# arkworks-rs/groth16

Measured on AMD Instinct MI355X. Metric: R1CS constraints/sec (create_proof, BLS12-381), higher is better.
Workload: dtype u32-limb Montgomery integers (Fr 255-bit, Fq 381-bit); 1 GPU; SYN(k=22) synthetic R1CS, 4194302 constraints, FFT domain 2^22, bls12_381, full create_proof (7 NTTs + 4 G1 MSMs + 1 G2 MSM), valid proving key generated on the GPU from seeded toxic waste; curve=bls12_381, log2_domain=22, constraints=4194302, key=valid, witness=resident in HBM at entry (--full: value_incl_h2d holds the PCIe-inclusive rates), parallelism=single-gpu

## Files before the change

### groth16_amd/csrc/internal.hpp

```cpp
#pragma once
#include <hip/hip_runtime.h>
#include <atomic>
#include <cstdint>
#include <cstdio>
#include <cstring>
#include <string>
#include <vector>
#include "../../include/g16_mi355x.h"
#include "curve.hpp"

namespace g16 {

void set_last_error(const char* what, hipError_t e, const char* file, int line);

#define G16_HIP_TRY(expr)                                                     \
    do {                                                                      \
        hipError_t e__ = (expr);                                              \
        if (e__ != hipSuccess) {                                              \
            ::g16::set_last_error(#expr, e__, __FILE__, __LINE__);            \
            return e__ == hipErrorOutOfMemory ? G16_ERR_OOM : G16_ERR_HIP;    \
        }                                                                     \
    } while (0)

#define G16_TRY(expr)                  \
    do {                               \
        int rc__ = (expr);             \
        if (rc__ != G16_OK) return rc__; \
    } while (0)

#define G16_LAUNCH_CHECK() G16_HIP_TRY(hipGetLastError())

struct PerDeviceOnce {
    std::atomic<bool> done[64] = {};
    std::atomic<bool>& flag() {
        int dev = 0;
        (void)hipGetDevice(&dev);
        return done[dev & 63];
    }
};

struct Arena {
    struct Chunk { char* p; size_t cap; size_t used; };
    std::vector<Chunk> chunks;
    size_t min_chunk = (size_t)256 << 20;
    void reset() { for (auto& c : chunks) c.used = 0; }
    int alloc(size_t bytes, void** out);
    template <class T> int alloc_n(size_t n, T** out) { return alloc(n * sizeof(T), (void**)out); }
    void release();
    size_t total() const { size_t t = 0; for (auto& c : chunks) t += c.cap; return t; }
};

struct EventTimer {
    hipEvent_t a = nullptr, b = nullptr;
    bool used = false;
    int start(hipStream_t s) {
        if (!a) { G16_HIP_TRY(hipEventCreate(&a)); G16_HIP_TRY(hipEventCreate(&b)); }
        used = true;
        G16_HIP_TRY(hipEventRecord(a, s));
        return G16_OK;
    }
    int stop(hipStream_t s) { G16_HIP_TRY(hipEventRecord(b, s)); return G16_OK; }
    double ms() {
        if (!used) return 0.0;
        float t = 0.f;
        if (hipEventElapsedTime(&t, a, b) != hipSuccess) return 0.0;
        return (double)t;
    }
    void destroy() { if (a) { (void)hipEventDestroy(a); (void)hipEventDestroy(b); a = b = nullptr; } }
};

template <class C>
struct Domain {
    typedef typename C::Fr Fr;
    int log_n = 0;
    size_t n = 0;
    Fr* tw_fwd = nullptr;
    Fr* tw_inv = nullptr;
    Fr* s1_br = nullptr;
    Fr* s2 = nullptr;
    Fr* g_pow = nullptr;
    Fr n_inv, zinv;
};
template <class C> int domain_create(int log_n, hipStream_t st, Domain<C>** out, bool coset_tables = true);
template <class C> void domain_destroy(Domain<C>* d);
template <class C> int domain_ensure_gpow(Domain<C>* d, hipStream_t st);

template <class C> int ntt_dif(const Domain<C>* d, typename C::Fr* data, bool inverse, hipStream_t st);
template <class C> int ntt_dif_quotient(const Domain<C>* d, typename C::Fr* a, const typename C::Fr* b, const typename C::Fr* c,
                                        const typename C::Fr& zinv, bool inverse, hipStream_t st);
template <class C> int ntt_dit(const Domain<C>* d, typename C::Fr* data, bool inverse, const typename C::Fr* prescale, hipStream_t st);
template <class C> int ntt_dif_dit(const Domain<C>* d, typename C::Fr* data, bool dif_inverse, const typename C::Fr* prescale, hipStream_t st);
template <class C> int ntt_dif_batch(const Domain<C>* d, typename C::Fr* const* data, int nbatch, bool inverse, hipStream_t st);
template <class C> int ntt_dit_batch(const Domain<C>* d, typename C::Fr* const* data, int nbatch, bool inverse, const typename C::Fr* prescale,
                                     hipStream_t st);
template <class C> int ntt_dif_dit_batch(const Domain<C>* d, typename C::Fr* const* data, int nbatch, bool dif_inverse,
                                         const typename C::Fr* prescale, hipStream_t st);
template <class C> int bitrev_scale(const Domain<C>* d, typename C::Fr* out, const typename C::Fr* in, const typename C::Fr* table,
                                    const typename C::Fr* cst, hipStream_t st);
template <class C> int scale_by_table(typename C::Fr* data, const typename C::Fr* table, size_t n, hipStream_t st);
template <class C> int gen_power_table(typename C::Fr* out, size_t n, const typename C::Fr& base, const typename C::Fr& scale, bool r30_form,
                                       hipStream_t st);
template <class C> int gen_bitrev_power_table(typename C::Fr* out, int log_n, const typename C::Fr& base, const typename C::Fr& scale,
                                              hipStream_t st);

template <class C>
struct DeviceCircuit {
    typedef typename C::Fr Fr;
    uint64_t num_inputs = 0, num_constraints = 0, num_variables = 0;
    uint64_t* row_ptr[3] = {nullptr, nullptr, nullptr};
    uint32_t* col[3] = {nullptr, nullptr, nullptr};
    Fr* val[3] = {nullptr, nullptr, nullptr};
    uint64_t nnz[3] = {0, 0, 0};
    Domain<C>* dom = nullptr;
    static constexpr int Z_CHUNKS = 8;
    uint64_t need_col[Z_CHUNKS] = {};
    int qap = G16_QAP_LIBSNARK;
    Fr* circom_pre = nullptr;
    bool long_rows = false;
};
struct ZUpload {
    const void* host = nullptr;
    hipStream_t copy_stream = nullptr;
    hipEvent_t landed[8] = {};
    int pieces = 0;
};
template <class C> int mark_unit_coefficients(DeviceCircuit<C>* ck, hipStream_t st);
template <class C> int mark_unit_matrix(uint32_t* col, const typename C::Fr* val, uint64_t nnz, hipStream_t st);
template <class C> int witness_map_device(const DeviceCircuit<C>* ck, const typename C::Fr* d_z, typename C::Fr* d_h, Arena& arena,
                                          hipStream_t st, EventTimer* ntt_timers = nullptr, ZUpload* up = nullptr);

static constexpr size_t R1CS_CHECK_SCRATCH = 128;
template <class C> int r1cs_check_device(const DeviceCircuit<C>* ck, const typename C::Fr* d_z, void* d_scratch, hipStream_t st,
                                         g16_check_result* out);
template <class C> int r1cs_attach_c_device(DeviceCircuit<C>* ck, const g16_csr_view* c, hipStream_t st);
template <class C> int r1cs_check_host(const g16_csr_view abc[3], uint64_t num_constraints, const uint64_t* z, uint64_t n_assign,
                                       g16_check_result* out);

template <class C>
struct DistWm {
    typedef typename C::Fr Fr;
    int rank = 0, world = 1, log_world = 0;
    size_t M = 0, blk = 0;
    Domain<C>* dom_m = nullptr;
    Fr* tw1 = nullptr;
    Fr* sc_mid = nullptr;
    Fr* tw2 = nullptr;
    Fr* sc_out = nullptr;
    Fr wn_fwd[8], wn_inv[8];
    Fr zinv;
};
template <class C> int dwm_create(const DeviceCircuit<C>* ck, int rank, int world, hipStream_t st, DistWm<C>** out);
template <class C> void dwm_destroy(DistWm<C>* d);
template <class C> int dwm_stage(const DeviceCircuit<C>* ck, const DistWm<C>* dw, int stage, const typename C::Fr* d_z,
                                 typename C::Fr* const work[3], typename C::Fr* const recv[3], typename C::Fr* h_local, hipStream_t st);

struct MsmPlan {
    int c = 0;
    int W = 0;
    int groups = 0;
    bool merged = false;
    uint32_t B = 0;
    uint32_t Lmax = 0;
    int affine_levels = 0;
    uint32_t chunk = 0;
    uint32_t K[10];
    int shard_n = 1, shard_r = 0;
    uint32_t buckets() const { return B * (uint32_t)groups; }
    uint32_t G = 8;
    uint32_t chunk_buckets() const { return B >= G ? G : B; }
    uint32_t chunks() const { return B / chunk_buckets(); }
    int chunk_bits() const { int k = 0; while ((1u << k) < chunks()) ++k; return k; }
    int planes() const { return 2 + chunk_bits(); }
    int outputs() const { return groups * planes(); }
};
static constexpr int MSM_MAX_OUTPUTS = 256;
static constexpr int MSM_MERGED_MIN_C = 9, MSM_MERGED_MAX_C = 20;
static constexpr uint64_t MSM_MERGED_MAX_N = (uint64_t)1 << 26;
int make_msm_plan(uint64_t n, int scalar_bits, const uint32_t* modulus_words, int mod_nwords, int merged_c, MsmPlan* plan, int shard_n = 1,
                  int shard_r = 0);
int msm_window_override();
int merged_window_bits(uint64_t n, int scalar_bits, const uint32_t* modulus_words, int mod_nwords);
int msm_plan_windows(int c, int scalar_bits, const uint32_t* modulus_words, int mod_nwords);

static constexpr uint32_t HEAVY_PARTS = 16;
struct ScalarSort {
    MsmPlan plan;
    uint64_t n = 0;
    uint32_t* sorted = nullptr;
    uint32_t* offsets = nullptr;
    uint32_t* task_off = nullptr;
    uint32_t* heavy = nullptr;
    uint32_t max_tasks = 0;
    uint32_t max_segments = 0;
    uint64_t max_sorted = 0;
};
template <class C> int sort_scalars(const typename C::Fr* d_scalars, uint64_t n, int merged_c, Arena& arena, hipStream_t st, ScalarSort* out,
                                    int shard_n = 1, int shard_r = 0);
static constexpr int COEFF128_SWORDS = 7;
int coeffs128_plan(uint64_t n, MsmPlan* plan);
int sort_digit_planes(const MsmPlan& plan, const uint16_t* planes, uint64_t n, Arena& arena, hipStream_t st, ScalarSort* out);
int msm_slot_layout(const uint32_t* counts, uint32_t M, int R, uint32_t lseg, uint32_t* offsets, uint32_t* nparts, uint32_t* task_off,
                    uint32_t* heavy, uint32_t* block_sums, hipStream_t st);

template <class F>
struct MsmBuffers {
    void* partials = nullptr;
    void* chunk_out = nullptr;
    XYZZ<F>* window_sums = nullptr;
};
template <class F> int msm_bucket_pass(const Affine<F>* d_bases, int64_t shift, uint64_t base_count, const ScalarSort& ss, Arena& arena,
                                       hipStream_t st, MsmBuffers<F>* out, EventTimer* bucket_timer);
template <class F>
struct PassJob {
    const Affine<F>* bases;
    int64_t shift;
    uint64_t base_count;
    const ScalarSort* ss;
    MsmBuffers<F>* out;
};
template <class F> int msm_bucket_pass_batch(const PassJob<F>* jobs, int n, Arena& arena, hipStream_t st, EventTimer* bucket_timer);
template <class F> int msm_reduce(const MsmBuffers<F>& buf, const ScalarSort& ss, hipStream_t st);
template <class F> int msm_reduce_batch(const MsmBuffers<F>* const* bufs, const ScalarSort* const* sorts, int n, hipStream_t st, bool heavy_done);
template <class F> int msm_heavy_reduce(const MsmBuffers<F>& buf, const ScalarSort& ss, hipStream_t st);
template <class F> int msm_heavy_reduce_batch(const MsmBuffers<F>* const* bufs, const ScalarSort* const* sorts, int n, hipStream_t st);
template <class F> int convert_bases(Affine<F>* d_bases, uint64_t n, hipStream_t st);
template <class F> XYZZ<F> fold_windows(const XYZZ<F>* window_sums, const MsmPlan& plan);
template <class F> int build_window_tables(const Affine<F>* d_src, uint64_t n, int c, int W, Affine<F>* d_table, hipStream_t st, void* park = nullptr);
template <class F> size_t window_table_park_bytes(uint64_t n, int W);

template <class C>
int generate_parameters_device(hipStream_t st, Arena& arena, const g16_csr_view abc[3], uint64_t ni, uint64_t nc, uint64_t nv, int qap,
                               const g16_toxic_waste* tw, const uint64_t* g1_gen, const uint64_t* g2_gen, const g16_params_view* out);
template <class C>
int h_query_scalars_host(int qap, uint64_t domain_size, const uint64_t* t, const uint64_t* delta_inverse, uint64_t* out);
template <class C>
int qap_evaluations_host(const g16_csr_view abc[3], uint64_t ni, uint64_t nc, uint64_t nv, const uint64_t* t, uint64_t* a_out, uint64_t* b_out,
                         uint64_t* c_out, uint64_t* zt_out);

int serialize_points(int curve, int g2, int compressed, const uint64_t* points, uint64_t n, uint8_t* out);
int deserialize_points(int curve, int g2, int compressed, const uint8_t* in, uint64_t n, int validate, uint64_t* points_out);
uint64_t serialized_point_size(int curve, int g2, int compressed);

int pk_load_bytes(g16_ctx* ctx, int curve, int device, hipStream_t s, const uint8_t* bytes, uint64_t len, int compressed, int validate,
                  g16_pk** out, void* info_out, uint64_t info_size);

int mad_rate_device(hipStream_t st, double* mad_per_s);
template <class C> int synth_bases_device(int g2, uint64_t seed, uint64_t first, uint64_t n, void* out_dev, hipStream_t st);

}
```

### groth16_amd/csrc/ntt.hip

```cpp
#include "internal.hpp"
#include "fp30.hpp"

namespace g16 {

#ifndef G16_NTT_TILE_LOG
#define G16_NTT_TILE_LOG 10
#endif
static constexpr int NTT_TILE_LOG = G16_NTT_TILE_LOG;
static constexpr int NTT_TILE = 1 << NTT_TILE_LOG;
#ifdef G16_NTT_THREADS
static constexpr int NTT_THREADS = G16_NTT_THREADS;
#else
static constexpr int NTT_THREADS = NTT_TILE_LOG >= 12 ? 512 : 256;
#endif
#ifndef G16_NTT_MAX_R
#define G16_NTT_MAX_R 2
#endif
static constexpr int NTT_MAX_R = G16_NTT_MAX_R;
#ifndef G16_NTT_MIN_WAVES
#define G16_NTT_MIN_WAVES 4
#endif
static constexpr int NTT_MAX_STRIDED = NTT_TILE_LOG >= 12 ? 10 : 8;
static constexpr int NTT_ROW = NTT_TILE + NTT_TILE / 32;

template <class Fr>
struct PowTable { Fr p[32]; };

template <class P>
struct Tw { uint32_t w[Fp30<P>::NL]; };
template <class P>
__device__ __forceinline__ Fp30<P> load_tw(const Tw<P>& e) {
    Fp30<P> r;
    G16_UNROLL for (int i = 0; i < Fp30<P>::NL; ++i) r.l[i] = e.w[i];
    return r;
}
template <class P>
__global__ void tw_convert_kernel(const Fp<P>* __restrict__ in, Tw<P>* __restrict__ out, size_t n) {
    const size_t i = (size_t)blockIdx.x * blockDim.x + threadIdx.x;
    if (i >= n) return;
    Tw<P> e;
    const Fp30<P> x = Fp30<P>::unpack(in[i].v);
    G16_UNROLL for (int k = 0; k < Fp30<P>::NL; ++k) e.w[k] = x.l[k];
    out[i] = e;
}

__device__ __forceinline__ uint32_t bitrev32(uint32_t x, int bits) { return bits ? (__brev(x) >> (32 - bits)) : 0u; }
__device__ __forceinline__ uint32_t lds_col(uint32_t e) { return e + (e >> 5); }

template <class Fr>
__global__ void gen_powers_kernel(Fr* __restrict__ out, size_t n, PowTable<Fr> tab, Fr scale, int rev_bits, int layered_log) {
    size_t i = (size_t)blockIdx.x * blockDim.x + threadIdx.x;
    if (i >= n) return;
    uint32_t e = rev_bits ? bitrev32((uint32_t)i, rev_bits) : (uint32_t)i;
    if (layered_log > 0) {
        const int s = 31 - __clz((uint32_t)i + 1u);
        e = (((uint32_t)i + 1u) - (1u << s)) << (layered_log - 1 - s);
    }
    Fr acc = scale;
    for (int j = 0; j < 32; ++j) {
        if ((e >> j) & 1) acc = acc * tab.p[j];
    }
    out[i] = acc;
}

template <class P, bool DIT, int R, class GIdx>
__device__ __forceinline__ void ntt30_round(uint32_t* lds, const Tw<P>* __restrict__ tw, int log_n, int s_lo, int q0, int TT, uint32_t E,
                                            int done, const GIdx& gidx, bool unit0) {
    typedef Fp30<P> F;
    constexpr int NL = F::NL;
    constexpr int NE = 1 << R;
    const int p0 = q0 + TT;
    for (uint32_t g = threadIdx.x; g < (E >> R); g += NTT_THREADS) {
        const uint32_t low = g & ((1u << p0) - 1), high = g >> p0;
        const uint32_t ebase = (high << (p0 + R)) | low;
        F x[NE];
        G16_UNROLL for (int j = 0; j < NE; ++j) {
            const uint32_t c = lds_col(ebase | ((uint32_t)j << p0));
            G16_UNROLL for (int l = 0; l < NL; ++l) x[j].l[l] = lds[l * NTT_ROW + c];
        }
        const uint64_t gbase = gidx(ebase);
        G16_UNROLL for (int qq = 0; qq < R; ++qq) {
            const int q = DIT ? qq : (R - 1 - qq);
            const int s = s_lo + q0 + q;
            const int kdone = done + qq;
            G16_UNROLL for (int j = 0; j < NE; ++j) {
                if (!((j >> q) & 1)) {
                    const int j2 = j | (1 << q);
                    const uint32_t gi = (uint32_t)gbase + ((uint32_t)j << (s_lo + q0));
                    const uint32_t widx = ((1u << s) - 1u) + (gi & ((1u << s) - 1u));
                    if (unit0 && s == 0) {
                        const F u = x[j], v = x[j2];
                        x[j] = u.add(v);
                        x[j2] = DIT ? u.template sub<2>(v) : u.sub_pow2(v, kdone);
                        continue;
                    }
                    const F w = load_tw<P>(tw[widx]);
                    if (DIT) {
                        const F v = x[j2].mul_impl(w);
                        const F u = x[j];
                        x[j] = u.add(v);
                        x[j2] = u.template sub<2>(v);
                    } else {
                        const F u = x[j], v = x[j2];
                        x[j] = u.add(v);
                        x[j2] = u.sub_pow2(v, kdone).mul_impl(w);
                    }
                }
            }
        }
        G16_UNROLL for (int j = 0; j < NE; ++j) {
            const uint32_t c = lds_col(ebase | ((uint32_t)j << p0));
            G16_UNROLL for (int l = 0; l < NL; ++l) lds[l * NTT_ROW + c] = x[j].l[l];
        }
    }
}

template <class P>
struct NttBatch { Fp<P>* p[3]; };
template <class P>
struct NttQuot { const Fp<P>* b; const Fp<P>* c; Fp<P> zinv; };

template <class P, bool DIT>
__global__ __launch_bounds__(NTT_THREADS, G16_NTT_MIN_WAVES) void ntt30_pass_kernel(NttBatch<P> batch, const Tw<P>* __restrict__ tw,
                                                                 const Fp<P>* __restrict__ prescale, int log_n, int s_lo, int s_hi,
                                                                 int T, NttQuot<P> quot) {
    typedef Fp30<P> F;
    constexpr int NL = F::NL;
    extern __shared__ __attribute__((aligned(16))) unsigned char smem[];
    uint32_t* lds = reinterpret_cast<uint32_t*>(smem);
    Fp<P>* __restrict__ data = batch.p[blockIdx.y];
    const int K = s_hi - s_lo;
    const int TT = (s_lo == 0) ? 0 : T;
    const uint32_t E = 1u << (K + TT);
    const uint64_t blk = blockIdx.x;
    uint64_t base;
    if (s_lo == 0) {
        base = blk << K;
    } else {
        const int mid_bits = s_lo - T;
        const uint64_t lowpart = blk & ((1ull << mid_bits) - 1);
        const uint64_t hipart = blk >> mid_bits;
        base = (lowpart << T) | (hipart << s_hi);
    }
    auto gidx = [&](uint32_t e) -> uint64_t {
        if (s_lo == 0) return base + e;
        const uint32_t low = e & ((1u << T) - 1), mid = e >> T;
        return base + low + ((uint64_t)mid << s_lo);
    };
    auto lds_load = [&](uint32_t e) -> F {
        F x;
        const uint32_t c = lds_col(e);
        G16_UNROLL for (int l = 0; l < NL; ++l) x.l[l] = lds[l * NTT_ROW + c];
        return x;
    };
    auto lds_store = [&](uint32_t e, const F& x) {
        const uint32_t c = lds_col(e);
        G16_UNROLL for (int l = 0; l < NL; ++l) lds[l * NTT_ROW + c] = x.l[l];
    };
    for (uint32_t e = threadIdx.x; e < E; e += NTT_THREADS) {
        const uint64_t g = gidx(e);
        F x;
        if (quot.b) {
            const Fp<P> t = (data[g] * quot.b[g] - quot.c[g]) * quot.zinv;
            x = F::unpack(t.v);
        } else {
            x = F::unpack(data[g].v);
        }
        if (prescale) x = x.mul_impl(F::unpack(prescale[g].v));
        lds_store(e, x);
    }
    __syncthreads();
    int done = 0;
    while (done < K) {
        const int R = (K - done) >= NTT_MAX_R ? NTT_MAX_R : (K - done);
        const int q0 = DIT ? done : (K - done - R);
        if (R == 3) ntt30_round<P, DIT, 3>(lds, tw, log_n, s_lo, q0, TT, E, done, gidx, true);
        else if (R == 2) ntt30_round<P, DIT, 2>(lds, tw, log_n, s_lo, q0, TT, E, done, gidx, true);
        else ntt30_round<P, DIT, 1>(lds, tw, log_n, s_lo, q0, TT, E, done, gidx, true);
        __syncthreads();
        done += R;
    }
    for (uint32_t e = threadIdx.x; e < E; e += NTT_THREADS) {
        const F x = lds_load(e).canonical_quick();
        Fp<P> o;
        x.pack(o.v);
        data[gidx(e)] = o;
    }
}

template <class P>
__global__ __launch_bounds__(NTT_THREADS, G16_NTT_MIN_WAVES) void ntt30_dif_dit_kernel(NttBatch<P> batch, const Tw<P>* __restrict__ tw_dif,
                                                                    const Tw<P>* __restrict__ tw_dit, const Fp<P>* __restrict__ prescale,
                                                                    int log_n, int K) {
    typedef Fp30<P> F;
    constexpr int NL = F::NL;
    extern __shared__ __attribute__((aligned(16))) unsigned char smem[];
    uint32_t* lds = reinterpret_cast<uint32_t*>(smem);
    Fp<P>* __restrict__ data = batch.p[blockIdx.y];
    const uint32_t E = 1u << K;
    const uint64_t base = (uint64_t)blockIdx.x << K;
    auto gidx = [&](uint32_t e) -> uint64_t { return base + e; };
    for (uint32_t e = threadIdx.x; e < E; e += NTT_THREADS) {
        const F x = F::unpack(data[base + e].v);
        const uint32_t c = lds_col(e);
        G16_UNROLL for (int l = 0; l < NL; ++l) lds[l * NTT_ROW + c] = x.l[l];
    }
    __syncthreads();
    for (int done = 0; done < K;) {
        const int R = (K - done) >= NTT_MAX_R ? NTT_MAX_R : (K - done);
        const int q0 = K - done - R;
        if (R == 3) ntt30_round<P, false, 3>(lds, tw_dif, log_n, 0, q0, 0, E, done, gidx, true);
        else if (R == 2) ntt30_round<P, false, 2>(lds, tw_dif, log_n, 0, q0, 0, E, done, gidx, true);
        else ntt30_round<P, false, 1>(lds, tw_dif, log_n, 0, q0, 0, E, done, gidx, true);
        __syncthreads();
        done += R;
    }
    if (prescale) {
        for (uint32_t e = threadIdx.x; e < E; e += NTT_THREADS) {
            const uint32_t c = lds_col(e);
            F x;
            G16_UNROLL for (int l = 0; l < NL; ++l) x.l[l] = lds[l * NTT_ROW + c];
            x = x.mul_impl(F::unpack(prescale[base + e].v));
            G16_UNROLL for (int l = 0; l < NL; ++l) lds[l * NTT_ROW + c] = x.l[l];
        }
        __syncthreads();
    }
    for (int done = 0; done < K;) {
        const int R = (K - done) >= NTT_MAX_R ? NTT_MAX_R : (K - done);
        const bool unit0 = prescale != nullptr;
        if (R == 3) ntt30_round<P, true, 3>(lds, tw_dit, log_n, 0, done, 0, E, done, gidx, unit0);
        else if (R == 2) ntt30_round<P, true, 2>(lds, tw_dit, log_n, 0, done, 0, E, done, gidx, unit0);
        else ntt30_round<P, true, 1>(lds, tw_dit, log_n, 0, done, 0, E, done, gidx, unit0);
        __syncthreads();
        done += R;
    }
    for (uint32_t e = threadIdx.x; e < E; e += NTT_THREADS) {
        const uint32_t c = lds_col(e);
        F x;
        G16_UNROLL for (int l = 0; l < NL; ++l) x.l[l] = lds[l * NTT_ROW + c];
        Fp<P> o;
        x.canonical_quick().pack(o.v);
        data[base + e] = o;
    }
}

template <class P>
__global__ void bitrev_scale_kernel(Fp<P>* __restrict__ out, const Fp<P>* __restrict__ in, const Fp<P>* __restrict__ table, Fp<P> cst,
                                    int has_cst, int log_n) {
    typedef Fp30<P> F;
    size_t k = (size_t)blockIdx.x * blockDim.x + threadIdx.x;
    if (k >= ((size_t)1 << log_n)) return;
    Fp<P> o = in[bitrev32((uint32_t)k, log_n)];
    if (table || has_cst) {
        F x = F::unpack(o.v);
        if (table) x = x.mul_impl(F::unpack(table[k].v));
        if (has_cst) x = x.mul_impl(F::unpack(cst.v));
        x.canonical_lt2p().pack(o.v);
    }
    out[k] = o;
}

template <class P>
__global__ void scale_table_kernel(Fp<P>* __restrict__ data, const Fp<P>* __restrict__ table, size_t n) {
    typedef Fp30<P> F;
    size_t k = (size_t)blockIdx.x * blockDim.x + threadIdx.x;
    if (k >= n) return;
    Fp<P> o;
    F::unpack(data[k].v).mul_impl(F::unpack(table[k].v)).canonical_lt2p().pack(o.v);
    data[k] = o;
}

struct PassPlan { int s_lo, s_hi, T; };

static std::vector<PassPlan> plan_passes(int log_n) {
    std::vector<PassPlan> p;
    if (log_n <= NTT_TILE_LOG) {
        p.push_back({0, log_n, 0});
        return p;
    }
    p.push_back({0, NTT_TILE_LOG, 0});
    int rest = log_n - NTT_TILE_LOG;
    const int npass = (rest + NTT_MAX_STRIDED - 1) / NTT_MAX_STRIDED;
    int s = NTT_TILE_LOG;
    for (int i = 0; i < npass; ++i) {
        const int left = npass - i;
        const int k = (rest + left - 1) / left;
        p.push_back({s, s + k, NTT_TILE_LOG - k});
        s += k;
        rest -= k;
    }
    return p;
}

template <class P, bool DIT>
static int launch_pass(const NttBatch<P>& batch, int nbatch, const Tw<P>* tw, const Fp<P>* prescale, int log_n, const PassPlan& pp, hipStream_t st,
                       const NttQuot<P>* quot = nullptr) {
    const int K = pp.s_hi - pp.s_lo;
    const int TT = pp.s_lo == 0 ? 0 : pp.T;
    const size_t E = (size_t)1 << (K + TT);
    const size_t blocks = ((size_t)1 << log_n) / E;
    const size_t lds_bytes = (size_t)Fp30<P>::NL * NTT_ROW * sizeof(uint32_t);
    static PerDeviceOnce attr_once;
    std::atomic<bool>& attr_set = attr_once.flag();
    if (!attr_set) {
        G16_HIP_TRY(hipFuncSetAttribute(reinterpret_cast<const void*>(&ntt30_pass_kernel<P, DIT>),
                                        hipFuncAttributeMaxDynamicSharedMemorySize, (int)lds_bytes));
        attr_set = true;
    }
    NttQuot<P> q;
    if (quot) q = *quot;
    else { q.b = nullptr; q.c = nullptr; q.zinv = Fp<P>::zero(); }
    hipLaunchKernelGGL((ntt30_pass_kernel<P, DIT>), dim3((unsigned)blocks, (unsigned)nbatch), dim3(NTT_THREADS), lds_bytes, st, batch, tw, prescale,
                       log_n, pp.s_lo, pp.s_hi, pp.T, q);
    G16_LAUNCH_CHECK();
    return G16_OK;
}

template <class C>
static NttBatch<typename C::Fr::Params> make_batch(typename C::Fr* const* data, int nbatch) {
    NttBatch<typename C::Fr::Params> b;
    for (int i = 0; i < 3; ++i) b.p[i] = data[i < nbatch ? i : 0];
    return b;
}

template <class C>
int ntt_dif_batch(const Domain<C>* d, typename C::Fr* const* data, int nbatch, bool inverse, hipStream_t st) {
    typedef typename C::Fr::Params P;
    if (nbatch < 1 || nbatch > 3) return G16_ERR_INTERNAL;
    if (d->log_n == 0) return G16_OK;
    auto passes = plan_passes(d->log_n);
    const Tw<P>* tw = reinterpret_cast<const Tw<P>*>(inverse ? d->tw_inv : d->tw_fwd);
    const NttBatch<P> b = make_batch<C>(data, nbatch);
    for (size_t i = passes.size(); i-- > 0;) G16_TRY((launch_pass<P, false>(b, nbatch, tw, nullptr, d->log_n, passes[i], st)));
    return G16_OK;
}
template <class C>
int ntt_dif(const Domain<C>* d, typename C::Fr* data, bool inverse, hipStream_t st) { return ntt_dif_batch<C>(d, &data, 1, inverse, st); }

template <class C>
int ntt_dif_quotient(const Domain<C>* d, typename C::Fr* a, const typename C::Fr* b, const typename C::Fr* c, const typename C::Fr& zinv,
                     bool inverse, hipStream_t st) {
    typedef typename C::Fr::Params P;
    auto passes = plan_passes(d->log_n);
    const Tw<P>* tw = reinterpret_cast<const Tw<P>*>(inverse ? d->tw_inv : d->tw_fwd);
    typename C::Fr* data[1] = {a};
    const NttBatch<P> batch = make_batch<C>(data, 1);
    NttQuot<P> q;
    q.b = b; q.c = c; q.zinv = zinv;
    if (d->log_n == 0) return G16_ERR_INTERNAL;
    for (size_t i = passes.size(); i-- > 0;)
        G16_TRY((launch_pass<P, false>(batch, 1, tw, nullptr, d->log_n, passes[i], st, i + 1 == passes.size() ? &q : nullptr)));
    return G16_OK;
}

template <class C>
int ntt_dit_batch(const Domain<C>* d, typename C::Fr* const* data, int nbatch, bool inverse, const typename C::Fr* prescale, hipStream_t st) {
    typedef typename C::Fr::Params P;
    if (nbatch < 1 || nbatch > 3) return G16_ERR_INTERNAL;
    if (d->log_n == 0) {
        if (prescale) for (int i = 0; i < nbatch; ++i) G16_TRY((scale_by_table<C>(data[i], prescale, 1, st)));
        return G16_OK;
    }
    auto passes = plan_passes(d->log_n);
    const Tw<P>* tw = reinterpret_cast<const Tw<P>*>(inverse ? d->tw_inv : d->tw_fwd);
    const NttBatch<P> b = make_batch<C>(data, nbatch);
    for (size_t i = 0; i < passes.size(); ++i)
        G16_TRY((launch_pass<P, true>(b, nbatch, tw, i == 0 ? prescale : nullptr, d->log_n, passes[i], st)));
    return G16_OK;
}
template <class C>
int ntt_dit(const Domain<C>* d, typename C::Fr* data, bool inverse, const typename C::Fr* prescale, hipStream_t st) {
    return ntt_dit_batch<C>(d, &data, 1, inverse, prescale, st);
}

template <class C>
int ntt_dif_dit_batch(const Domain<C>* d, typename C::Fr* const* data, int nbatch, bool dif_inverse, const typename C::Fr* prescale, hipStream_t st) {
    typedef typename C::Fr::Params P;
    if (nbatch < 1 || nbatch > 3) return G16_ERR_INTERNAL;
    if (d->log_n == 0) {
        if (prescale) for (int i = 0; i < nbatch; ++i) G16_TRY((scale_by_table<C>(data[i], prescale, 1, st)));
        return G16_OK;
    }
    auto passes = plan_passes(d->log_n);
    const Tw<P>* tw1 = reinterpret_cast<const Tw<P>*>(dif_inverse ? d->tw_inv : d->tw_fwd);
    const Tw<P>* tw2 = reinterpret_cast<const Tw<P>*>(dif_inverse ? d->tw_fwd : d->tw_inv);
    const NttBatch<P> b = make_batch<C>(data, nbatch);
    for (size_t i = passes.size(); i-- > 1;) G16_TRY((launch_pass<P, false>(b, nbatch, tw1, nullptr, d->log_n, passes[i], st)));
    {
        const int K = passes[0].s_hi;
        const size_t blocks = ((size_t)1 << d->log_n) >> K;
        const size_t lds_bytes = (size_t)Fp30<P>::NL * NTT_ROW * sizeof(uint32_t);
        static PerDeviceOnce attr_once;
        std::atomic<bool>& attr_set = attr_once.flag();
        if (!attr_set) {
            G16_HIP_TRY(hipFuncSetAttribute(reinterpret_cast<const void*>(&ntt30_dif_dit_kernel<P>), hipFuncAttributeMaxDynamicSharedMemorySize,
                                            (int)lds_bytes));
            attr_set = true;
        }
        hipLaunchKernelGGL((ntt30_dif_dit_kernel<P>), dim3((unsigned)blocks, (unsigned)nbatch), dim3(NTT_THREADS), lds_bytes, st, b, tw1, tw2, prescale,
                           d->log_n, K);
        G16_LAUNCH_CHECK();
    }
    for (size_t i = 1; i < passes.size(); ++i) G16_TRY((launch_pass<P, true>(b, nbatch, tw2, nullptr, d->log_n, passes[i], st)));
    return G16_OK;
}
template <class C>
int ntt_dif_dit(const Domain<C>* d, typename C::Fr* data, bool dif_inverse, const typename C::Fr* prescale, hipStream_t st) {
    return ntt_dif_dit_batch<C>(d, &data, 1, dif_inverse, prescale, st);
}

template <class C>
int bitrev_scale(const Domain<C>* d, typename C::Fr* out, const typename C::Fr* in, const typename C::Fr* table,
                 const typename C::Fr* cst, hipStream_t st) {
    typedef typename C::Fr Fr;
    const size_t n = d->n;
    Fr c = cst ? *cst : Fr::zero();
    hipLaunchKernelGGL((bitrev_scale_kernel<typename Fr::Params>), dim3((unsigned)((n + 255) / 256)), dim3(256), 0, st, out, in, table, c,
                       cst ? 1 : 0, d->log_n);
    G16_LAUNCH_CHECK();
    return G16_OK;
}

template <class C>
int scale_by_table(typename C::Fr* data, const typename C::Fr* table, size_t n, hipStream_t st) {
    typedef typename C::Fr Fr;
    hipLaunchKernelGGL((scale_table_kernel<typename Fr::Params>), dim3((unsigned)((n + 255) / 256)), dim3(256), 0, st, data, table, n);
    G16_LAUNCH_CHECK();
    return G16_OK;
}

template <class Fr>
static int gen_powers30(Fr* out, size_t n, const Fr& base, const Fr& scale, int rev_bits, hipStream_t st, int layered_log = 0) {
    if (n == 0) return G16_OK;
    PowTable<Fr> tab;
    Fr p = base;
    for (int j = 0; j < 32; ++j) { tab.p[j] = p; p = p.sqr(); }
    const Fr scale30 = Fp30<typename Fr::Params>::std_to_r30(scale);
    hipLaunchKernelGGL((gen_powers_kernel<Fr>), dim3((unsigned)((n + 255) / 256)), dim3(256), 0, st, out, n, tab, scale30, rev_bits, layered_log);
    G16_LAUNCH_CHECK();
    return G16_OK;
}

template <class C>
int gen_power_table(typename C::Fr* out, size_t n, const typename C::Fr& base, const typename C::Fr& scale, bool r30_form, hipStream_t st) {
    typedef typename C::Fr Fr;
    if (r30_form) return gen_powers30<Fr>(out, n, base, scale, 0, st);
    if (n == 0) return G16_OK;
    PowTable<Fr> tab;
    Fr p = base;
    for (int j = 0; j < 32; ++j) { tab.p[j] = p; p = p.sqr(); }
    hipLaunchKernelGGL((gen_powers_kernel<Fr>), dim3((unsigned)((n + 255) / 256)), dim3(256), 0, st, out, n, tab, scale, 0, 0);
    G16_LAUNCH_CHECK();
    return G16_OK;
}

template <class C>
int gen_bitrev_power_table(typename C::Fr* out, int log_n, const typename C::Fr& base, const typename C::Fr& scale, hipStream_t st) {
    return gen_powers30<typename C::Fr>(out, (size_t)1 << log_n, base, scale, log_n, st);
}

template <class C>
int domain_create(int log_n, hipStream_t st, Domain<C>** out, bool coset_tables) {
    typedef typename C::Fr Fr;
    if (log_n > C::TWO_ADICITY || log_n > 31) return G16_ERR_DEGREE_TOO_LARGE;
    Domain<C>* d = new Domain<C>();
    d->log_n = log_n;
    d->n = (size_t)1 << log_n;
    const size_t n = d->n;
    Fr omega = C::two_adic_root();
    for (int i = log_n; i < C::TWO_ADICITY; ++i) omega = omega.sqr();
    Fr omega_inv = omega.inverse();
    const Fr n_inv = Fr::from_u64((uint64_t)n).inverse();
    d->n_inv = Fp30<typename Fr::Params>::std_to_r30(n_inv);
    const Fr g = C::fr_generator(), g_inv = C::fr_generator_inv();
    d->zinv = (g.pow_u64((uint64_t)n) - Fr::one()).inverse();
    int rc = G16_OK;
    const size_t ntw = n > 1 ? n - 1 : 1;
    typedef Tw<typename Fr::Params> TwE;
    Fr* tw_tmp = nullptr;
    auto fail = [&](int code) {
        (void)hipStreamSynchronize(st);
        (void)hipFree(tw_tmp);
        domain_destroy<C>(d);
        return code;
    };
    if (hipMalloc((void**)&d->tw_fwd, ntw * sizeof(TwE)) != hipSuccess) return fail(G16_ERR_OOM);
    if (hipMalloc((void**)&d->tw_inv, ntw * sizeof(TwE)) != hipSuccess) return fail(G16_ERR_OOM);
    if (hipMalloc((void**)&tw_tmp, ntw * sizeof(Fr)) != hipSuccess) return fail(G16_ERR_OOM);
    if (coset_tables && hipMalloc((void**)&d->s1_br, n * sizeof(Fr)) != hipSuccess) return fail(G16_ERR_OOM);
    if (coset_tables && hipMalloc((void**)&d->s2, n * sizeof(Fr)) != hipSuccess) return fail(G16_ERR_OOM);
    for (int dir = 0; dir < 2; ++dir) {
        if ((rc = gen_powers30<Fr>(tw_tmp, ntw, dir ? omega_inv : omega, Fr::one(), 0, st, log_n)) != G16_OK) return fail(rc);
        hipLaunchKernelGGL((tw_convert_kernel<typename Fr::Params>), dim3((unsigned)((ntw + 255) / 256)), dim3(256), 0, st, tw_tmp,
                           reinterpret_cast<TwE*>(dir ? d->tw_inv : d->tw_fwd), ntw);
        if (hipGetLastError() != hipSuccess) return fail(G16_ERR_HIP);
    }
    if (coset_tables && (rc = gen_powers30<Fr>(d->s1_br, n, g, n_inv, log_n, st)) != G16_OK) return fail(rc);
    if (coset_tables && (rc = gen_powers30<Fr>(d->s2, n, g_inv, n_inv, 0, st)) != G16_OK) return fail(rc);
    if (hipStreamSynchronize(st) != hipSuccess) return fail(G16_ERR_HIP);
    (void)hipFree(tw_tmp);
    *out = d;
    return G16_OK;
}

template <class C>
int domain_ensure_gpow(Domain<C>* d, hipStream_t st) {
    typedef typename C::Fr Fr;
    if (d->g_pow) return G16_OK;
    G16_HIP_TRY(hipMalloc((void**)&d->g_pow, d->n * sizeof(Fr)));
    return gen_powers30<Fr>(d->g_pow, d->n, C::fr_generator(), Fr::one(), 0, st);
}

template <class C>
void domain_destroy(Domain<C>* d) {
    if (!d) return;
    (void)hipFree(d->tw_fwd); (void)hipFree(d->tw_inv); (void)hipFree(d->s1_br); (void)hipFree(d->s2); (void)hipFree(d->g_pow);
    delete d;
}

#define G16_INSTANTIATE_NTT(C)                                                                                     \
    template int domain_create<C>(int, hipStream_t, Domain<C>**, bool);                                            \
    template int gen_bitrev_power_table<C>(typename C::Fr*, int, const typename C::Fr&, const typename C::Fr&, hipStream_t); \
    template void domain_destroy<C>(Domain<C>*);                                                                   \
    template int domain_ensure_gpow<C>(Domain<C>*, hipStream_t);                                                   \
    template int ntt_dif<C>(const Domain<C>*, typename C::Fr*, bool, hipStream_t);                                 \
    template int ntt_dif_quotient<C>(const Domain<C>*, typename C::Fr*, const typename C::Fr*, const typename C::Fr*, const typename C::Fr&, bool, hipStream_t); \
    template int ntt_dit<C>(const Domain<C>*, typename C::Fr*, bool, const typename C::Fr*, hipStream_t);          \
    template int ntt_dif_dit<C>(const Domain<C>*, typename C::Fr*, bool, const typename C::Fr*, hipStream_t);      \
    template int ntt_dif_batch<C>(const Domain<C>*, typename C::Fr* const*, int, bool, hipStream_t);              \
    template int ntt_dit_batch<C>(const Domain<C>*, typename C::Fr* const*, int, bool, const typename C::Fr*, hipStream_t);   \
    template int ntt_dif_dit_batch<C>(const Domain<C>*, typename C::Fr* const*, int, bool, const typename C::Fr*, hipStream_t); \
    template int bitrev_scale<C>(const Domain<C>*, typename C::Fr*, const typename C::Fr*, const typename C::Fr*,  \
                                 const typename C::Fr*, hipStream_t);                                              \
    template int scale_by_table<C>(typename C::Fr*, const typename C::Fr*, size_t, hipStream_t);                   \
    template int gen_power_table<C>(typename C::Fr*, size_t, const typename C::Fr&, const typename C::Fr&, bool, hipStream_t);

G16_INSTANTIATE_NTT(Bls12_381)
G16_INSTANTIATE_NTT(Bn254)

}
```

### groth16_amd/csrc/witness_map.hip

```cpp
#include "internal.hpp"
#include "csr_row_dot.hpp"
#include <algorithm>
#include <new>

namespace g16 {

template <class Fr>
struct SpmvArgs {
    const uint64_t* row_ptr[3];
    const uint32_t* col[3];
    const Fr* val[3];
    Fr* out[3];
};

template <class Fr>
__global__ void spmv3_kernel(SpmvArgs<Fr> args, const Fr* __restrict__ z, uint64_t num_inputs, uint64_t nc, uint64_t row0, uint64_t stride,
                             uint64_t rows, int out_rev_bits, uint64_t out0) {
    const int m = blockIdx.y;
    const uint64_t li = (uint64_t)blockIdx.x * blockDim.x + threadIdx.x;
    if (li >= rows) return;
    const uint64_t row = row0 + stride * li;
    Fr acc = Fr::zero();
    if (row < nc) {
        const uint64_t b = args.row_ptr[m][row], e = args.row_ptr[m][row + 1];
// ... 9 lines not shown
            }
        }
    } else if (m == 0 && row - nc < num_inputs) {
        acc = z[row - nc];
    }
    args.out[m][out0 + (out_rev_bits ? (uint64_t)(__brev((uint32_t)li) >> (32 - out_rev_bits)) : li)] = acc;
}

template <class Fr>
__global__ void quotient_kernel(Fr* __restrict__ a, const Fr* __restrict__ b, const Fr* __restrict__ c, Fr zinv, size_t n) {
    size_t i = (size_t)blockIdx.x * blockDim.x + threadIdx.x;
    if (i >= n) return;
    a[i] = (a[i] * b[i] - c[i]) * zinv;
}


template <class Fr>
struct CircomSpmvArgs {
    const uint64_t* row_ptr[2];
    const uint32_t* col[2];
    const Fr* val[2];
    Fr* out[3];
};
template <class Fr>
__global__ __launch_bounds__(256) void spmv_circom_kernel(CircomSpmvArgs<Fr> args, const Fr* __restrict__ z, uint64_t num_inputs, uint64_t nc, uint64_t row0,
                                   uint64_t rows) {
    const uint32_t li = blockIdx.x * blockDim.x + threadIdx.x;
    if (li >= rows) return;
    const uint32_t row = (uint32_t)row0 + li;
    if (row < nc) {
#pragma unroll 1
        for (int m = 0; m < 2; ++m) args.out[m][row] = csr_row_dot<Fr>(args.row_ptr[m], args.col[m], args.val[m], z, row);
        args.out[2][row] = args.out[0][row] * args.out[1][row];
    } else {
        args.out[0][row] = (row - nc < num_inputs) ? z[row - nc] : Fr::zero();
        args.out[1][row] = Fr::zero();
        args.out[2][row] = Fr::zero();
    }
}

template <class Fr>
__global__ void circom_h_kernel(Fr* __restrict__ h, const Fr* __restrict__ a, const Fr* __restrict__ b, const Fr* __restrict__ c, size_t n) {
    const size_t i = (size_t)blockIdx.x * blockDim.x + threadIdx.x;
    if (i >= n) return;
    h[i] = a[i] * b[i] - c[i];
}

template <class C>
static int launch_spmv_circom(const DeviceCircuit<C>* ck, const typename C::Fr* d_z, typename C::Fr* a, typename C::Fr* b, typename C::Fr* c,
                              uint64_t row0, uint64_t rows, hipStream_t st) {
    typedef typename C::Fr Fr;
    if (!rows) return G16_OK;
    CircomSpmvArgs<Fr> args;
    for (int m = 0; m < 2; ++m) {
        args.row_ptr[m] = ck->row_ptr[m];
        args.col[m] = ck->col[m];
        args.val[m] = ck->val[m];
    }
    args.out[0] = a; args.out[1] = b; args.out[2] = c;
    hipLaunchKernelGGL((spmv_circom_kernel<Fr>), dim3((unsigned)((rows + 255) / 256)), dim3(256), 0, st, args, d_z, ck->num_inputs,
                       ck->num_constraints, row0, rows);
    G16_LAUNCH_CHECK();
    return G16_OK;
}

template <class C, class LaunchRows>
static int upload_pieces_and_rows(const DeviceCircuit<C>* ck, const typename C::Fr* d_z, size_t n, hipStream_t st, ZUpload* up, LaunchRows launch_rows) {
    typedef typename C::Fr Fr;
    constexpr int ZC = DeviceCircuit<C>::Z_CHUNKS;
    const uint64_t nz = ck->num_variables;
    const int pieces = (int)std::min<uint64_t>(4, std::max<uint64_t>(1, nz >> 16));
    up->pieces = pieces;
    const uint64_t per = (nz + pieces - 1) / pieces;
    for (int k = 0; k < pieces; ++k) {
        const uint64_t lo = per * k, hi = std::min(nz, per * (k + 1));
        if (hi > lo)
            G16_HIP_TRY(hipMemcpyAsync(const_cast<Fr*>(d_z) + lo, static_cast<const Fr*>(up->host) + lo, (hi - lo) * sizeof(Fr),
                                       hipMemcpyHostToDevice, up->copy_stream));
        G16_HIP_TRY(hipEventRecord(up->landed[k], up->copy_stream));
    }
    int next_block = 0;
    for (int k = 0; k < pieces; ++k) {
        const uint64_t hi = std::min(nz, per * (k + 1));
        int last_block = next_block;
        while (last_block < ZC && (k == pieces - 1 || ck->need_col[last_block] < hi)) ++last_block;
        if (last_block > next_block) {
            const uint64_t r_lo = n * (uint64_t)next_block / ZC, r_hi = n * (uint64_t)last_block / ZC;
            G16_HIP_TRY(hipStreamWaitEvent(st, up->landed[k], 0));
            if (r_hi > r_lo) G16_TRY(launch_rows(r_lo, r_hi - r_lo));
            next_block = last_block;
        }
    }
    return G16_OK;
}

template <class C>
static int witness_map_circom(const DeviceCircuit<C>* ck, const typename C::Fr* d_z, typename C::Fr* d_h, Arena& arena, hipStream_t st,
                              EventTimer* ntt_timers, ZUpload* up) {
    typedef typename C::Fr Fr;
    const Domain<C>* dom = ck->dom;
    const size_t n = dom->n;
    Fr *a = nullptr, *b = nullptr, *c = nullptr;
    G16_TRY(arena.alloc_n(n, &a));
    G16_TRY(arena.alloc_n(n, &b));
    G16_TRY(arena.alloc_n(n, &c));
    Fr* outs[3] = {a, b, c};
    if (!up) {
        G16_TRY((launch_spmv_circom<C>(ck, d_z, a, b, c, 0, n, st)));
    } else {
        G16_TRY((upload_pieces_and_rows<C>(ck, d_z, n, st, up, [&](uint64_t r0, uint64_t rows) -> int { return launch_spmv_circom<C>(ck, d_z, a, b, c, r0, rows, st); })));
    }
    if (ntt_timers) {
        ntt_timers[1].used = false;
        G16_TRY(ntt_timers[0].start(st));
    }
    if (dom->log_n > 0) G16_TRY((ntt_dif_dit_batch<C>(dom, outs, 3, true, ck->circom_pre, st)));
    if (ntt_timers) G16_TRY(ntt_timers[0].stop(st));
    hipLaunchKernelGGL((circom_h_kernel<Fr>), dim3((unsigned)((n + 255) / 256)), dim3(256), 0, st, d_h, a, b, c, n);
    G16_LAUNCH_CHECK();
    return G16_OK;
}

template <class C>
int witness_map_device(const DeviceCircuit<C>* ck, const typename C::Fr* d_z, typename C::Fr* d_h, Arena& arena, hipStream_t st,
                       EventTimer* ntt_timers, ZUpload* up) {
    typedef typename C::Fr Fr;
    if (ck->qap == G16_QAP_CIRCOM) return witness_map_circom<C>(ck, d_z, d_h, arena, st, ntt_timers, up);
    const Domain<C>* dom = ck->dom;
    const size_t n = dom->n;
    Fr *a = nullptr, *b = nullptr, *c = nullptr;
    G16_TRY(arena.alloc_n(n, &a));
    G16_TRY(arena.alloc_n(n, &b));
    G16_TRY(arena.alloc_n(n, &c));
    SpmvArgs<Fr> args;
    Fr* outs[3] = {a, b, c};
    for (int m = 0; m < 3; ++m) {
        args.row_ptr[m] = ck->row_ptr[m];
        args.col[m] = ck->col[m];
        args.val[m] = ck->val[m];
        args.out[m] = outs[m];
    }
    if (!up) {
        hipLaunchKernelGGL((spmv3_kernel<Fr>), dim3((unsigned)((n + 255) / 256), 3), dim3(256), 0, st, args, d_z, ck->num_inputs,
                           ck->num_constraints, (uint64_t)0, (uint64_t)1, (uint64_t)n, 0, (uint64_t)0);
        G16_LAUNCH_CHECK();
    } else {
        G16_TRY((upload_pieces_and_rows<C>(ck, d_z, n, st, up, [&](uint64_t r0, uint64_t rows) -> int {
            hipLaunchKernelGGL((spmv3_kernel<Fr>), dim3((unsigned)((rows + 255) / 256), 3), dim3(256), 0, st, args, d_z, ck->num_inputs,
                               ck->num_constraints, r0, (uint64_t)1, rows, 0, r0);
            G16_LAUNCH_CHECK();
            return G16_OK;
        })));
    }
    if (ntt_timers) G16_TRY(ntt_timers[0].start(st));
    G16_TRY((ntt_dif_dit_batch<C>(dom, outs, 3, true, dom->s1_br, st)));
    if (ntt_timers) G16_TRY(ntt_timers[0].stop(st));
    if (ntt_timers) G16_TRY(ntt_timers[1].start(st));
    if (dom->log_n == 0) {
        hipLaunchKernelGGL((quotient_kernel<Fr>), dim3((unsigned)((n + 255) / 256)), dim3(256), 0, st, a, b, c, dom->zinv, n);
        G16_LAUNCH_CHECK();
    } else {
        G16_TRY((ntt_dif_quotient<C>(dom, a, b, c, dom->zinv, true, st)));
    }
    G16_TRY((bitrev_scale<C>(dom, d_h, a, dom->s2, nullptr, st)));
    if (ntt_timers) G16_TRY(ntt_timers[1].stop(st));
    return G16_OK;
}

template <class Fr>
struct SmallRoots { Fr w[8]; };

template <class Fr, int LOGN>
__device__ __forceinline__ void dft_small(Fr* v, const SmallRoots<Fr>& roots) {
    constexpr int N = 1 << LOGN;
    G16_UNROLL for (int s = LOGN - 1; s >= 0; --s) {
        const int half = 1 << s;
        G16_UNROLL for (int i = 0; i < N; ++i) {
            if (i & half) continue;
            const int k = (i & (half - 1)) << (LOGN - 1 - s);
            const Fr u = v[i], t = v[i + half];
            v[i] = u + t;
            v[i + half] = k ? (u - t) * roots.w[k] : (u - t);
        }
    }
    G16_UNROLL for (int i = 0; i < N; ++i) {
        int j = 0;
        G16_UNROLL for (int b = 0; b < LOGN; ++b) j |= ((i >> b) & 1) << (LOGN - 1 - b);
        if (j > i) { const Fr t = v[i]; v[i] = v[j]; v[j] = t; }
    }
}

template <class Fr, int LOGN, bool TWO>
__global__ __launch_bounds__(128) void dwm_column_kernel(const Fr* __restrict__ in0, const Fr* __restrict__ in1, const Fr* __restrict__ in2, Fr* __restrict__ out0,
                                  Fr* __restrict__ out1, Fr* __restrict__ out2, size_t blk, SmallRoots<Fr> roots_a, const Fr* __restrict__ sc_a,
                                  SmallRoots<Fr> roots_b, const Fr* __restrict__ sc_b) {
    constexpr int N = 1 << LOGN;
    const size_t j = (size_t)blockIdx.x * blockDim.x + threadIdx.x;
    if (j >= blk) return;
    const Fr* in = blockIdx.y == 0 ? in0 : blockIdx.y == 1 ? in1 : in2;
    Fr* out = blockIdx.y == 0 ? out0 : blockIdx.y == 1 ? out1 : out2;
    Fr v[N];
    G16_UNROLL for (int i = 0; i < N; ++i) v[i] = in[(size_t)i * blk + j];
    dft_small<Fr, LOGN>(v, roots_a);
    G16_UNROLL for (int i = 0; i < N; ++i) v[i] = v[i] * sc_a[(size_t)i * blk + j];
    if (TWO) {
        dft_small<Fr, LOGN>(v, roots_b);
        G16_UNROLL for (int i = 0; i < N; ++i) v[i] = v[i] * sc_b[(size_t)i * blk + j];
    }
    G16_UNROLL for (int i = 0; i < N; ++i) out[(size_t)i * blk + j] = v[i];
}

template <class C>
void dwm_destroy(DistWm<C>* d) {
    if (!d) return;
    (void)hipFree(d->tw1); (void)hipFree(d->sc_mid); (void)hipFree(d->tw2); (void)hipFree(d->sc_out);
    domain_destroy<C>(d->dom_m);
    delete d;
}

template <class C>
int dwm_create(const DeviceCircuit<C>* ck, int rank, int world, hipStream_t st, DistWm<C>** out) {
    typedef typename C::Fr Fr;
    if (ck->qap != G16_QAP_LIBSNARK) return G16_ERR_BAD_ARG;
    const int log_n = ck->dom->log_n;
    int lw = 0;
    while ((1 << lw) < world) ++lw;
    if (world < 1 || world > 16 || (1 << lw) != world || rank < 0 || rank >= world) return G16_ERR_BAD_ARG;
    if (2 * lw > log_n) return G16_ERR_BAD_LENGTH;
    DistWm<C>* d = new (std::nothrow) DistWm<C>();
    if (!d) return G16_ERR_OOM;
    d->rank = rank; d->world = world; d->log_world = lw;
    d->M = (size_t)1 << (log_n - lw);
    d->blk = d->M >> lw;
    auto fail = [&](int code) { dwm_destroy<C>(d); return code; };
    int rc = domain_create<C>(log_n - lw, st, &d->dom_m);
    if (rc) return fail(rc);
    const size_t M = d->M, blk = d->blk, N = (size_t)world;
    Fr omega = C::two_adic_root();
    for (int i = log_n; i < C::TWO_ADICITY; ++i) omega = omega.sqr();
    const Fr omega_inv = omega.inverse();
    const Fr n_inv = Fr::from_u64((uint64_t)1 << log_n).inverse();
    const Fr g = C::fr_generator(), g_inv = C::fr_generator_inv();
    if (hipMalloc((void**)&d->tw1, M * sizeof(Fr)) != hipSuccess || hipMalloc((void**)&d->sc_mid, M * sizeof(Fr)) != hipSuccess ||
        hipMalloc((void**)&d->tw2, M * sizeof(Fr)) != hipSuccess || hipMalloc((void**)&d->sc_out, M * sizeof(Fr)) != hipSuccess)
        return fail(G16_ERR_OOM);
    const uint64_t r = (uint64_t)rank;
    if ((rc = gen_power_table<C>(d->tw1, M, omega_inv.pow_u64(r), Fr::one(), true, st))) return fail(rc);
    for (uint64_t k = 0; k < N; ++k) {
        const uint64_t e0 = r * blk + (uint64_t)M * k;
        if ((rc = gen_power_table<C>(d->sc_mid + k * blk, blk, g, n_inv * g.pow_u64(e0), false, st))) return fail(rc);
        if ((rc = gen_power_table<C>(d->sc_out + k * blk, blk, g_inv, n_inv * g_inv.pow_u64(e0), false, st))) return fail(rc);
        const Fr wk = omega.pow_u64(k);
        if ((rc = gen_power_table<C>(d->tw2 + k * blk, blk, wk, wk.pow_u64(r * blk), false, st))) return fail(rc);
    }
    const Fr wN = omega.pow_u64((uint64_t)M), wN_inv = omega_inv.pow_u64((uint64_t)M);
    for (int k = 0; k < 8; ++k) { d->wn_fwd[k] = wN.pow_u64((uint64_t)k); d->wn_inv[k] = wN_inv.pow_u64((uint64_t)k); }
    d->zinv = ck->dom->zinv;
    if (hipStreamSynchronize(st) != hipSuccess) return fail(G16_ERR_HIP);
    *out = d;
    return G16_OK;
}

template <class C, bool TWO>
static int dwm_columns(const DistWm<C>* d, int chains, typename C::Fr* const in[3], typename C::Fr* const outp[3], const typename C::Fr* sc_a,
                       const typename C::Fr* sc_b, hipStream_t st) {
    typedef typename C::Fr Fr;
    SmallRoots<Fr> ra, rb;
    for (int k = 0; k < 8; ++k) { ra.w[k] = d->wn_inv[k]; rb.w[k] = d->wn_fwd[k]; }
    const dim3 grid((unsigned)((d->blk + 127) / 128), (unsigned)chains), block(128);
#define G16_DWM_LAUNCH(LOGN)                                                                                                          \
    hipLaunchKernelGGL((dwm_column_kernel<Fr, LOGN, TWO>), grid, block, 0, st, in[0], in[1], in[2], outp[0], outp[1], outp[2], d->blk, ra, sc_a, \
                       rb, sc_b)
    switch (d->log_world) {
        case 0: G16_DWM_LAUNCH(0); break;
        case 1: G16_DWM_LAUNCH(1); break;
        case 2: G16_DWM_LAUNCH(2); break;
        case 3: G16_DWM_LAUNCH(3); break;
        case 4: G16_DWM_LAUNCH(4); break;
        default: return G16_ERR_INTERNAL;
    }
#undef G16_DWM_LAUNCH
    G16_LAUNCH_CHECK();
    return G16_OK;
}

template <class C>
int dwm_stage(const DeviceCircuit<C>* ck, const DistWm<C>* d, int stage, const typename C::Fr* d_z, typename C::Fr* const work[3],
              typename C::Fr* const recv[3], typename C::Fr* h_local, hipStream_t st) {
    typedef typename C::Fr Fr;
    const Domain<C>* dm = d->dom_m;
    const size_t M = d->M;
    if (stage == 0) {
        SpmvArgs<Fr> args;
        for (int m = 0; m < 3; ++m) {
            args.row_ptr[m] = ck->row_ptr[m];
            args.col[m] = ck->col[m];
            args.val[m] = ck->val[m];
            args.out[m] = work[m];
        }
        hipLaunchKernelGGL((spmv3_kernel<Fr>), dim3((unsigned)((M + 255) / 256), 3), dim3(256), 0, st, args, d_z, ck->num_inputs,
                           ck->num_constraints, (uint64_t)d->rank, (uint64_t)d->world, (uint64_t)M, dm->log_n, (uint64_t)0);
        G16_LAUNCH_CHECK();
        G16_TRY((ntt_dit_batch<C>(dm, work, 3, true, nullptr, st)));
        for (int m = 0; m < 3; ++m) G16_TRY((scale_by_table<C>(work[m], d->tw1, M, st)));
        return G16_OK;
    }
    if (stage == 1) {
        return dwm_columns<C, true>(d, 3, recv, work, d->sc_mid, d->tw2, st);
    }
    if (stage == 2) {
        G16_TRY((ntt_dif_batch<C>(dm, recv, 3, false, st)));
        hipLaunchKernelGGL((quotient_kernel<Fr>), dim3((unsigned)((M + 255) / 256)), dim3(256), 0, st, recv[0], recv[1], recv[2], d->zinv, M);
        G16_LAUNCH_CHECK();
        G16_HIP_TRY(hipMemcpyAsync(work[0], recv[0], M * sizeof(Fr), hipMemcpyDeviceToDevice, st));
        G16_TRY((ntt_dit<C>(dm, work[0], true, nullptr, st)));
        G16_TRY((scale_by_table<C>(work[0], d->tw1, M, st)));
        return G16_OK;
// ... 47 lines not shown
```

Before: 69.72 million constraints/s.

## Skip C coset round-trip by exploiting INTT linearity in quotient

New measurement: 70.26 million constraints/s, median of 6. About the same (+0.8%).

```diff
diff --git a/groth16_amd/csrc/internal.hpp b/groth16_amd/csrc/internal.hpp
--- a/groth16_amd/csrc/internal.hpp
+++ b/groth16_amd/csrc/internal.hpp
@@ -80,6 +80,7 @@
     Fr* s2 = nullptr;
     Fr* g_pow = nullptr;
     Fr n_inv, zinv;
+    Fr zinv_n_inv;
 };
 template <class C> int domain_create(int log_n, hipStream_t st, Domain<C>** out, bool coset_tables = true);
 template <class C> void domain_destroy(Domain<C>* d);
@@ -87,7 +88,7 @@
 
 template <class C> int ntt_dif(const Domain<C>* d, typename C::Fr* data, bool inverse, hipStream_t st);
 template <class C> int ntt_dif_quotient(const Domain<C>* d, typename C::Fr* a, const typename C::Fr* b, const typename C::Fr* c,
-                                        const typename C::Fr& zinv, bool inverse, hipStream_t st);
+                                        const typename C::Fr& zinv, bool inverse, hipStream_t st, typename C::Fr* also = nullptr);
 template <class C> int ntt_dit(const Domain<C>* d, typename C::Fr* data, bool inverse, const typename C::Fr* prescale, hipStream_t st);
 template <class C> int ntt_dif_dit(const Domain<C>* d, typename C::Fr* data, bool dif_inverse, const typename C::Fr* prescale, hipStream_t st);
 template <class C> int ntt_dif_batch(const Domain<C>* d, typename C::Fr* const* data, int nbatch, bool inverse, hipStream_t st);
@@ -96,7 +97,8 @@
 template <class C> int ntt_dif_dit_batch(const Domain<C>* d, typename C::Fr* const* data, int nbatch, bool dif_inverse,
                                          const typename C::Fr* prescale, hipStream_t st);
 template <class C> int bitrev_scale(const Domain<C>* d, typename C::Fr* out, const typename C::Fr* in, const typename C::Fr* table,
-                                    const typename C::Fr* cst, hipStream_t st);
+                                    const typename C::Fr* cst, hipStream_t st, const typename C::Fr* in2 = nullptr,
+                                    const typename C::Fr* cst2 = nullptr);
 template <class C> int scale_by_table(typename C::Fr* data, const typename C::Fr* table, size_t n, hipStream_t st);
 template <class C> int gen_power_table(typename C::Fr* out, size_t n, const typename C::Fr& base, const typename C::Fr& scale, bool r30_form,
                                        hipStream_t st);
diff --git a/groth16_amd/csrc/ntt.hip b/groth16_amd/csrc/ntt.hip
--- a/groth16_amd/csrc/ntt.hip
+++ b/groth16_amd/csrc/ntt.hip
@@ -160,8 +160,10 @@
     for (uint32_t e = threadIdx.x; e < E; e += NTT_THREADS) {
         const uint64_t g = gidx(e);
         F x;
-        if (quot.b) {
-            const Fp<P> t = (data[g] * quot.b[g] - quot.c[g]) * quot.zinv;
+        if (quot.b && blockIdx.y == 0) {
+            Fp<P> t = data[g] * quot.b[g];
+            if (quot.c) t = t - quot.c[g];
+            t = t * quot.zinv;
             x = F::unpack(t.v);
         } else {
             x = F::unpack(data[g].v);
@@ -246,16 +248,24 @@
 
 template <class P>
 __global__ void bitrev_scale_kernel(Fp<P>* __restrict__ out, const Fp<P>* __restrict__ in, const Fp<P>* __restrict__ table, Fp<P> cst,
-                                    int has_cst, int log_n) {
+                                    int has_cst, int log_n, const Fp<P>* __restrict__ in2, Fp<P> cst2) {
     typedef Fp30<P> F;
     size_t k = (size_t)blockIdx.x * blockDim.x + threadIdx.x;
+    if (log_n >= 8)
+        k = (size_t)(threadIdx.x & 15u) | ((size_t)blockIdx.x << 4) | ((size_t)(__brev(threadIdx.x >> 4) >> 28) << (log_n - 4));
     if (k >= ((size_t)1 << log_n)) return;
-    Fp<P> o = in[bitrev32((uint32_t)k, log_n)];
+    const uint32_t r = bitrev32((uint32_t)k, log_n);
+    Fp<P> o = in[r];
     if (table || has_cst) {
         F x = F::unpack(o.v);
         if (table) x = x.mul_impl(F::unpack(table[k].v));
         if (has_cst) x = x.mul_impl(F::unpack(cst.v));
         x.canonical_lt2p().pack(o.v);
+    }
+    if (in2) {
+        Fp<P> s;
+        F::unpack(in2[r].v).mul_impl(F::unpack(cst2.v)).canonical_lt2p().pack(s.v);
+        o = o - s;
     }
     out[k] = o;
 }
@@ -339,17 +349,18 @@
 
 template <class C>
 int ntt_dif_quotient(const Domain<C>* d, typename C::Fr* a, const typename C::Fr* b, const typename C::Fr* c, const typename C::Fr& zinv,
-                     bool inverse, hipStream_t st) {
+                     bool inverse, hipStream_t st, typename C::Fr* also) {
     typedef typename C::Fr::Params P;
     auto passes = plan_passes(d->log_n);
     const Tw<P>* tw = reinterpret_cast<const Tw<P>*>(inverse ? d->tw_inv : d->tw_fwd);
-    typename C::Fr* data[1] = {a};
-    const NttBatch<P> batch = make_batch<C>(data, 1);
+    typename C::Fr* data[2] = {a, also};
+    const int nbatch = also ? 2 : 1;
+    const NttBatch<P> batch = make_batch<C>(data, nbatch);
     NttQuot<P> q;
     q.b = b; q.c = c; q.zinv = zinv;
     if (d->log_n == 0) return G16_ERR_INTERNAL;
     for (size_t i = passes.size(); i-- > 0;)
-        G16_TRY((launch_pass<P, false>(batch, 1, tw, nullptr, d->log_n, passes[i], st, i + 1 == passes.size() ? &q : nullptr)));
+        G16_TRY((launch_pass<P, false>(batch, nbatch, tw, nullptr, d->log_n, passes[i], st, i + 1 == passes.size() ? &q : nullptr)));
     return G16_OK;
 }
 
@@ -411,12 +422,14 @@
 
 template <class C>
 int bitrev_scale(const Domain<C>* d, typename C::Fr* out, const typename C::Fr* in, const typename C::Fr* table,
-                 const typename C::Fr* cst, hipStream_t st) {
+                 const typename C::Fr* cst, hipStream_t st, const typename C::Fr* in2, const typename C::Fr* cst2) {
     typedef typename C::Fr Fr;
     const size_t n = d->n;
+    if ((in2 != nullptr) != (cst2 != nullptr)) return G16_ERR_INTERNAL;
     Fr c = cst ? *cst : Fr::zero();
+    Fr c2 = cst2 ? *cst2 : Fr::zero();
     hipLaunchKernelGGL((bitrev_scale_kernel<typename Fr::Params>), dim3((unsigned)((n + 255) / 256)), dim3(256), 0, st, out, in, table, c,
-                       cst ? 1 : 0, d->log_n);
+                       cst ? 1 : 0, d->log_n, in2, c2);
     G16_LAUNCH_CHECK();
     return G16_OK;
 }
@@ -474,6 +487,7 @@
     d->n_inv = Fp30<typename Fr::Params>::std_to_r30(n_inv);
     const Fr g = C::fr_generator(), g_inv = C::fr_generator_inv();
     d->zinv = (g.pow_u64((uint64_t)n) - Fr::one()).inverse();
+    d->zinv_n_inv = Fp30<typename Fr::Params>::std_to_r30(d->zinv * n_inv);
     int rc = G16_OK;
     const size_t ntw = n > 1 ? n - 1 : 1;
     typedef Tw<typename Fr::Params> TwE;
@@ -524,14 +538,15 @@
     template void domain_destroy<C>(Domain<C>*);                                                                   \
     template int domain_ensure_gpow<C>(Domain<C>*, hipStream_t);                                                   \
     template int ntt_dif<C>(const Domain<C>*, typename C::Fr*, bool, hipStream_t);                                 \
-    template int ntt_dif_quotient<C>(const Domain<C>*, typename C::Fr*, const typename C::Fr*, const typename C::Fr*, const typename C::Fr&, bool, hipStream_t); \
+    template int ntt_dif_quotient<C>(const Domain<C>*, typename C::Fr*, const typename C::Fr*, const typename C::Fr*, const typename C::Fr&, bool, hipStream_t, \
+                                     typename C::Fr*);                                                             \
     template int ntt_dit<C>(const Domain<C>*, typename C::Fr*, bool, const typename C::Fr*, hipStream_t);          \
     template int ntt_dif_dit<C>(const Domain<C>*, typename C::Fr*, bool, const typename C::Fr*, hipStream_t);      \
     template int ntt_dif_batch<C>(const Domain<C>*, typename C::Fr* const*, int, bool, hipStream_t);              \
     template int ntt_dit_batch<C>(const Domain<C>*, typename C::Fr* const*, int, bool, const typename C::Fr*, hipStream_t);   \
     template int ntt_dif_dit_batch<C>(const Domain<C>*, typename C::Fr* const*, int, bool, const typename C::Fr*, hipStream_t); \
     template int bitrev_scale<C>(const Domain<C>*, typename C::Fr*, const typename C::Fr*, const typename C::Fr*,  \
-                                 const typename C::Fr*, hipStream_t);                                              \
+                                 const typename C::Fr*, hipStream_t, const typename C::Fr*, const typename C::Fr*); \
     template int scale_by_table<C>(typename C::Fr*, const typename C::Fr*, size_t, hipStream_t);                   \
     template int gen_power_table<C>(typename C::Fr*, size_t, const typename C::Fr&, const typename C::Fr&, bool, hipStream_t);
 
diff --git a/groth16_amd/csrc/witness_map.hip b/groth16_amd/csrc/witness_map.hip
--- a/groth16_amd/csrc/witness_map.hip
+++ b/groth16_amd/csrc/witness_map.hip
@@ -185,17 +185,23 @@
             return G16_OK;
         })));
     }
+    if (dom->log_n == 0) {
+        if (ntt_timers) G16_TRY(ntt_timers[0].start(st));
+        G16_TRY((ntt_dif_dit_batch<C>(dom, outs, 3, true, dom->s1_br, st)));
+        if (ntt_timers) G16_TRY(ntt_timers[0].stop(st));
+        if (ntt_timers) G16_TRY(ntt_timers[1].start(st));
+        hipLaunchKernelGGL((quotient_kernel<Fr>), dim3((unsigned)((n + 255) / 256)), dim3(256), 0, st, a, b, c, dom->zinv, n);
+        G16_LAUNCH_CHECK();
+        G16_TRY((bitrev_scale<C>(dom, d_h, a, dom->s2, nullptr, st)));
+        if (ntt_timers) G16_TRY(ntt_timers[1].stop(st));
+        return G16_OK;
+    }
     if (ntt_timers) G16_TRY(ntt_timers[0].start(st));
-    G16_TRY((ntt_dif_dit_batch<C>(dom, outs, 3, true, dom->s1_br, st)));
+    G16_TRY((ntt_dif_dit_batch<C>(dom, outs, 2, true, dom->s1_br, st)));
     if (ntt_timers) G16_TRY(ntt_timers[0].stop(st));
     if (ntt_timers) G16_TRY(ntt_timers[1].start(st));
-    if (dom->log_n == 0) {
-        hipLaunchKernelGGL((quotient_kernel<Fr>), dim3((unsigned)((n + 255) / 256)), dim3(256), 0, st, a, b, c, dom->zinv, n);
-        G16_LAUNCH_CHECK();
-    } else {
-        G16_TRY((ntt_dif_quotient<C>(dom, a, b, c, dom->zinv, true, st)));
-    }
-    G16_TRY((bitrev_scale<C>(dom, d_h, a, dom->s2, nullptr, st)));
+    G16_TRY((ntt_dif_quotient<C>(dom, a, b, nullptr, dom->zinv, true, st, c)));
+    G16_TRY((bitrev_scale<C>(dom, d_h, a, dom->s2, nullptr, st, c, &dom->zinv_n_inv)));
     if (ntt_timers) G16_TRY(ntt_timers[1].stop(st));
     return G16_OK;
 }
```
